# lucagem29/mcmc_clv_model

Measured on AMD Instinct MI355X. Metric: MCMC sweeps/sec x N_customers (customer-sweeps/s), higher is better.
Workload: dtype f64

## Files before the change

include/clvmcmc.h:

```cpp
#ifndef CLVMCMC_H
#define CLVMCMC_H

#include <stdint.h>

#ifdef __cplusplus
extern "C" {
#endif

#define CLV_ABI_VERSION 2

#define CLV_BLOCK 256
#define CLV_MAX_K 9
#define CLV_MAX_D 3

enum { CLV_OK = 0, CLV_EINVAL = -1, CLV_EHIP = -2, CLV_ESTATE = -3, CLV_ENOMEM = -4 };
enum { CLV_RNG_PHILOX = 0, CLV_RNG_REPLAY = 1 };
enum { CLV_SINK_FULL = 0, CLV_SINK_SUMMARY = 1, CLV_SINK_NONE = 2, CLV_SINK_SUMMARY_PCT = 3 };

#define CLV_SUMMARY_MU_CAP 0.05
enum {
  CLV_SUM_LAMBDA = 0, CLV_SUM_MU, CLV_SUM_Z, CLV_SUM_LOG_LAMBDA, CLV_SUM_LOG_MU,
  CLV_SUM_LAMBDA2, CLV_SUM_MU2, CLV_SUM_ETA, CLV_SUM_LOG_ETA, CLV_SUM_MU_CAPPED, CLV_SUM_TAU,
  CLV_N_SUM_STATS
};
// ... 88 lines not shown
                  int64_t sweeps_done);

int clv_set_timing(clv_sampler* s, int32_t enable);
int clv_kernel_time(clv_sampler* s, double* sweep_kernel_ms_total, int64_t* sweep_launches,
                    double* hyper_kernel_ms_total, int64_t* hyper_launches);

int clv_debug_host_times(const clv_sampler* s, int64_t* out);
int clv_debug_philox(uint32_t k0, uint32_t k1, const uint32_t* ctr, int64_t n, uint32_t* out);
int clv_debug_variates(uint64_t seed, int32_t chain, uint32_t sweep, int64_t n, int32_t n_steps,
                       float* t_l, float* t_m, float* u_acc, double* u_z, double* u_tau,
                       double* e_alive, double* eta_z, float* log2_u_acc);
int clv_debug_log2u_scan(uint64_t w_begin, uint64_t w_end, double* out);
int clv_debug_t3(const uint32_t* words, int64_t n, int32_t packed, float* t_l, float* t_m);
int clv_debug_level2(int32_t D, int32_t K, const clv_prior* prior, const double* xty,
                     const double* yty, const double* iw_normal, const double* iw_chi2,
                     const double* z, double* beta, double* sigma);
int clv_debug_stamps(clv_sampler* s, uint64_t* out);
int clv_debug_wg_stamps(clv_sampler* s, uint64_t* out);
int clv_debug_hyper_variates(uint64_t seed, int32_t chain, uint32_t sweep, double df, int64_t n,
                             double* chi2, double* normals);
int clv_debug_exp(const double* x, int64_t n, double* out);
int clv_debug_log(const double* x, int64_t n, double* out);
int clv_debug_mh_step(int64_t n, const int32_t* x, const uint8_t* z, const double* T_cal, const double* tau,
                      const double* mean, const double* prec3, const double* cur_pt, const float* t3,
                      const double* scale2, const float* log_u, double* out);
int clv_debug_wg_map(int32_t n_chains, int32_t nb, int32_t n_cu, int32_t* out);
int clv_debug_persist_fits(int64_t grid_wgs, int32_t blocks_per_cu, int32_t n_cu);
int clv_debug_persist_choice(int32_t D, int32_t K, int32_t n_chains, int64_t grid_wgs, int32_t blocks_per_cu,
                             int32_t n_cu);
int clv_debug_split_fits(int32_t n_chains, int32_t nb, int32_t blocks_per_cu, int32_t n_cu);
int clv_debug_split_choice(int32_t n_chains, int32_t nb, int32_t blocks_per_cu, int32_t n_cu);
int clv_debug_split_layout(int32_t n_chains, int32_t nb, int32_t* out);
int clv_debug_split_relay_plan(int32_t S, int32_t R, int32_t* out);
int clv_debug_split_stamps(clv_sampler* s, uint64_t* out);

enum { CLV_EXCHANGE_AUTO = 0, CLV_EXCHANGE_P2P = 1, CLV_EXCHANGE_COPY = 2 };
typedef struct clv_group clv_group;
int clv_group_create(clv_sampler* const* shards, int32_t n, int32_t exchange, clv_group** out);
int clv_group_run(clv_group* g, int64_t n_sweeps);
int32_t clv_group_exchange(const clv_group* g);
void clv_group_destroy(clv_group* g);

enum {
  CLV_L1_MEAN_LAMBDA = 0, CLV_L1_LAMBDA_P025, CLV_L1_LAMBDA_P975, CLV_L1_MEAN_MU, CLV_L1_MEAN_MU_CAPPED,
  CLV_L1_MU_P025, CLV_L1_MU_P975, CLV_L1_MEAN_Z, CLV_L1_MEAN_TAU, CLV_L1_MEAN_ETA, CLV_N_L1_STATS
};
int clv_predict(int32_t device, const double* level1, int64_t n_draws, int64_t n, int32_t width,
                const double* T_cal, double T_star, uint64_t seed, int32_t simulate_spend, double sigma_s,
                int64_t* x_future, double* spend_future);
int clv_predict_sampler(clv_sampler* s, double T_star, uint64_t seed, int32_t simulate_spend,
                        double sigma_s, int64_t* x_future, double* spend_future);
int clv_track(int32_t device, const double* level1, int64_t n_draws, int64_t n, int32_t width,
              const double* birth_week, const double* times, int32_t n_times, uint64_t seed,
              double* inc_weekly);
int clv_track_sampler(clv_sampler* s, const double* birth_week, const double* times, int32_t n_times,
                      uint64_t seed, double* inc_weekly);
int clv_level1_summary(int32_t device, const double* level1, int64_t n_draws, int64_t n, int32_t width,
                       double mu_cap, double* out);
int clv_level1_summary_sampler(clv_sampler* s, double mu_cap, double* out);
int clv_chain_total_loglik(int32_t device, const double* level1, int64_t n_draws, int64_t n, int32_t width,
                           const int32_t* x, const double* T_cal, double* mean_total);
int clv_chain_total_loglik_sampler(clv_sampler* s, double* mean_total);

enum {
  CLV_LTV_VALUE_MEAN = 0, CLV_LTV_VALUE_SD, CLV_LTV_VALUE_P025, CLV_LTV_VALUE_P50, CLV_LTV_VALUE_P975,
  CLV_LTV_RESIDUAL_MEAN, CLV_LTV_RESIDUAL_SD, CLV_LTV_RESIDUAL_P025, CLV_LTV_RESIDUAL_P50, CLV_LTV_RESIDUAL_P975,
// ... 109 lines not shown
```

mcmc_clv_model_amd/_lib.py:

```python
from __future__ import annotations

import ctypes
import os
from ctypes import c_uint8, POINTER, c_char_p, c_double, c_float, c_int32, c_int64, c_uint32, c_uint64, c_void_p

try:
    import torch
except Exception:
    torch = None

LIB_NAME = "libclvmcmc.so"
LIB_PATH = os.environ.get("CLV_LIB_PATH") or os.path.join(os.path.dirname(os.path.abspath(__file__)), LIB_NAME)

ABI_VERSION = 2
BLOCK = 256
MAX_K = 9
MAX_D = 3
RNG_PHILOX, RNG_REPLAY = 0, 1
SINK_FULL, SINK_SUMMARY, SINK_NONE, SINK_SUMMARY_PCT = 0, 1, 2, 3
EXCHANGE_AUTO, EXCHANGE_P2P, EXCHANGE_COPY = 0, 1, 2
SUM_STATS = ("lambda", "mu", "z", "log_lambda", "log_mu", "lambda2", "mu2", "eta", "log_eta", "mu_capped", "tau")
SUMMARY_MU_CAP = 0.05
N_SUM_STATS = len(SUM_STATS)
TAPE_HYPER = 40
# ... 62 lines not shown
        "clv_synchronize": (c_int32, [sp]),
        "clv_sweeps_done": (c_int64, [sp]),
        "clv_clock_ghz": (c_int32, [sp, POINTER(c_double)]),
        "clv_clock_probe": (c_int32, [sp, c_double, POINTER(c_double)]),
        "clv_launch_info": (c_int32, [sp, POINTER(c_int64)]),
        "clv_split_relay_steps": (c_int32, [sp, POINTER(c_int32)]),
        "clv_p2p_info": (c_int32, [sp, POINTER(c_int64)]),
        "clv_p2p_export": (c_int32, [sp, c_void_p]),
        "clv_p2p_connect": (c_int32, [sp, c_void_p, POINTER(c_uint64)]),
        "clv_p2p_disconnect": (c_int32, [sp]),
        "clv_p2p_set_persistent": (c_int32, [sp, c_int32]),
        "clv_set_wait_timeout": (c_int32, [sp, c_double]),
        "clv_set_stream": (c_int32, [sp, c_uint64]),
        "clv_note_sweeps": (c_int32, [sp, c_int64]),
        "clv_read_draws": (c_int32, [sp, dp, dp, dp]),
        "clv_stream_draws": (c_int32, [sp, dp]),
        "clv_read_summary": (c_int32, [sp, dp, POINTER(c_int64)]),
        "clv_get_state": (c_int32, [sp, dp, dp, dp]),
        "clv_set_state": (c_int32, [sp, dp, dp, dp, c_int64]),
        "clv_set_timing": (c_int32, [sp, c_int32]),
        "clv_kernel_time": (c_int32, [sp, dp, POINTER(c_int64), dp, POINTER(c_int64)]),
        "clv_debug_philox": (c_int32, [c_uint32, c_uint32, POINTER(c_uint32), c_int64, POINTER(c_uint32)]),
        "clv_debug_variates": (c_int32, [c_uint64, c_int32, c_uint32, c_int64, c_int32, POINTER(c_float),
                                         POINTER(c_float), POINTER(c_float), dp, dp, dp, dp, POINTER(c_float)]),
        "clv_debug_log2u_scan": (c_int32, [c_uint64, c_uint64, dp]),
        "clv_debug_host_times": (c_int32, [sp, POINTER(c_int64)]),
        "clv_debug_t3": (c_int32, [POINTER(c_uint32), c_int64, c_int32, POINTER(c_float), POINTER(c_float)]),
        "clv_debug_level2": (c_int32, [c_int32, c_int32, POINTER(ClvPrior), dp, dp, dp, dp, dp, dp, dp]),
        "clv_debug_hyper_variates": (c_int32, [c_uint64, c_int32, c_uint32, c_double, c_int64, dp, dp]),
        "clv_debug_stamps": (c_int32, [sp, POINTER(c_uint64)]),
        "clv_debug_wg_stamps": (c_int32, [sp, POINTER(c_uint64)]),
        "clv_debug_split_stamps": (c_int32, [sp, POINTER(c_uint64)]),
        "clv_debug_split_relay_plan": (c_int32, [c_int32, c_int32, POINTER(c_int32)]),
        "clv_debug_exp": (c_int32, [dp, c_int64, dp]),
        "clv_debug_log": (c_int32, [dp, c_int64, dp]),
        "clv_debug_mh_step": (c_int32, [c_int64, POINTER(c_int32), POINTER(c_uint8), dp, dp, dp, dp, dp,
                                        POINTER(c_float), dp, POINTER(c_float), dp]),
        "clv_debug_wg_map": (c_int32, [c_int32, c_int32, c_int32, POINTER(c_int32)]),
        "clv_debug_persist_choice": (c_int32, [c_int32, c_int32, c_int32, c_int64, c_int32, c_int32]),
        "clv_debug_persist_fits": (c_int32, [c_int64, c_int32, c_int32]),
        "clv_group_create": (c_int32, [POINTER(sp), c_int32, c_int32, POINTER(sp)]),
        "clv_group_run": (c_int32, [sp, c_int64]),
        "clv_group_exchange": (c_int32, [sp]),
        "clv_group_destroy": (None, [sp]),
        "clv_predict": (c_int32, [c_int32, dp, c_int64, c_int64, c_int32, dp, c_double, c_uint64, c_int32, c_double,
                                  POINTER(c_int64), dp]),
        "clv_predict_sampler": (c_int32, [sp, c_double, c_uint64, c_int32, c_double, POINTER(c_int64), dp]),
        "clv_track": (c_int32, [c_int32, dp, c_int64, c_int64, c_int32, dp, dp, c_int32, c_uint64, dp]),
        "clv_track_sampler": (c_int32, [sp, dp, dp, c_int32, c_uint64, dp]),
        "clv_level1_summary": (c_int32, [c_int32, dp, c_int64, c_int64, c_int32, c_double, dp]),
        "clv_level1_summary_sampler": (c_int32, [sp, c_double, dp]),
        "clv_chain_total_loglik": (c_int32, [c_int32, dp, c_int64, c_int64, c_int32, POINTER(c_int32), dp, dp]),
        "clv_chain_total_loglik_sampler": (c_int32, [sp, dp]),
        "clv_lifetime_value": (c_int32, [c_int32, dp, c_int64, c_int64, c_int32, dp, c_double, c_double, c_double,
                                         c_double, dp, dp]),
        "clv_lifetime_value_sampler": (c_int32, [sp, dp, c_double, c_double, c_double, c_double, dp, dp]),
        "clv_ltv_info": (c_int32, [POINTER(c_int64)]),
        "clv_pointwise_loglik": (c_int32, [c_int32, dp, c_int64, c_int64, c_int32, POINTER(c_int32), dp, dp, dp,
                                           c_double, dp]),
        "clv_psis_loo": (c_int32, [c_int32, dp, c_int64, c_int64, c_double, dp]),
        "clv_information_criteria": (c_int32, [c_int32, dp, c_int64, c_int64, c_int32, POINTER(c_int32), dp, dp, dp,
                                               c_double, c_double, dp]),
        "clv_information_criteria_sampler": (c_int32, [sp, c_int32, c_double, c_double, dp]),
        "clv_ic_info": (c_int32, [POINTER(c_int64)]),
        "clv_debug_information_criteria": (c_int32, [c_int32, dp, c_int64, c_int64, c_int32, POINTER(c_int32), dp,
                                                     dp, dp, c_double, c_double, c_int64, c_int32, dp]),
# ... 126 lines not shown
```

mcmc_clv_model_amd/csrc/capi.hip:

```cpp
#include <hip/hip_runtime.h>

#include <algorithm>
#include <chrono>
#include <cstdlib>
#include <cstdio>
#include <cstring>
#include <string>
#include <vector>

#include "internal.h"
#include "kernels.h"
#include "philox.h"

using namespace clv;

namespace {

thread_local std::string g_err;

constexpr int PRIOR_DOUBLES = 81 + 81 + 27 + 9;
constexpr int GRAPH_CHUNK = 64;
constexpr int TIMING_EVENTS = 256;

}
// ... 1556 lines not shown
  CLV_HIP(hipMemcpy(chi2, dc, sizeof(double) * n, hipMemcpyDeviceToHost));
  CLV_HIP(hipMemcpy(normals, dn, sizeof(double) * n, hipMemcpyDeviceToHost));
  CLV_HIP(hipFree(dc));
  CLV_HIP(hipFree(dn));
  return CLV_OK;
}

int clv_debug_persist_choice(int32_t D, int32_t K, int32_t n_chains, int64_t grid_wgs, int32_t blocks_per_cu,
                             int32_t n_cu) {
  return persist_grid_fits(grid_wgs, blocks_per_cu, n_cu) && persist_worth(D, K, n_chains, grid_wgs, n_cu) ? 1 : 0;
}

int clv_debug_persist_fits(int64_t grid_wgs, int32_t blocks_per_cu, int32_t n_cu) {
  return persist_grid_fits(grid_wgs, blocks_per_cu, n_cu) ? 1 : 0;
}

int clv_debug_split_fits(int32_t n_chains, int32_t nb, int32_t blocks_per_cu, int32_t n_cu) {
  return persist_split_fits(n_chains, nb, blocks_per_cu, n_cu) ? 1 : 0;
}

int clv_debug_split_choice(int32_t n_chains, int32_t nb, int32_t blocks_per_cu, int32_t n_cu) {
  return persist_split_fits(n_chains, nb, blocks_per_cu, n_cu) && persist_split_pays(n_chains, nb, n_cu) ? 1 : 0;
}

int clv_debug_split_relay_plan(int32_t S, int32_t R, int32_t* out) {
  if (!out || S < 0 || S > PRE_STEPS || !(R == 0 || R == 8 || R == 12)) return fail(CLV_EINVAL, "bad arguments");
  const SplitRelayPlan pl = split_relay_plan(S, R);
  const int32_t o[8] = {pl.own_begin, pl.own_end, pl.relay_begin, pl.relay_end,
                        pl.own_begin, pl.own_end, pl.relay_begin, pl.relay_end};
  std::copy(o, o + 8, out);
  return CLV_OK;
}

int clv_debug_split_layout(int32_t n_chains, int32_t nb, int32_t* out) {
  if (!out || n_chains < 1 || nb < 1 || nb > SPLIT_MAX_NB || n_chains >= (1 << 15)) return fail(CLV_EINVAL, "bad arguments");
  const std::vector<int32_t> m = persist_split_layout(n_chains, nb);
  const int nwg = split_wgs(nb);
  for (size_t i = 0; i < m.size(); ++i) {
    int32_t* o = out + 8 * i;
    const int p = m[i] & 0xFFFF;
    o[0] = m[i] >> 16;
    for (int k = 1; k < 8; ++k) o[k] = -1;
    if (p == nwg) continue;
    const int r0 = SPLIT_CW * p;
    o[1] = r0;
    o[2] = std::min(SPLIT_CW, 4 * nb - r0);
    const int b0 = (p & 1) ? (r0 - 2) / 4 : r0 / 4, b1 = (p & 1) ? (r0 + 2) / 4 : r0 / 4 + 1;
    o[3] = (p & 1) ? 3 : 1;
    o[4] = b0;
    if (b1 < nb) {
      o[5] = (p & 1) ? 1 : 2;
      o[6] = b1;
    }
    o[7] = (p & 1) ? nb + 2 * (b0 / 3) : -1;
  }
  return CLV_OK;
}

int clv_debug_wg_map(int32_t n_chains, int32_t nb, int32_t n_cu, int32_t* out) {
  if (!out || n_chains < 1 || nb < 0 || n_cu < 1 || n_chains >= (1 << 15) || nb >= (1 << 16))
    return fail(CLV_EINVAL, "bad arguments");
  const std::vector<int32_t> m = persist_wg_map(n_chains, nb, n_cu);
  std::copy(m.begin(), m.end(), out);
  return CLV_OK;
}

// ... 58 lines not shown
```

mcmc_clv_model_amd/csrc/kernels.h:

```cpp
#pragma once
#include <hip/hip_runtime.h>
#include <stdint.h>

#include "../../include/clvmcmc.h"

namespace clv {

constexpr int BLOCK = CLV_BLOCK;
constexpr int HS = 64;
constexpr int H_TAG = 63;
constexpr int TAPE_HYPER = 40;
constexpr int MAX_WORLD = 64;
constexpr int UMAIL = 2048;
constexpr int HV = 40;
constexpr int MAIL_TAIL = MAX_WORLD;
constexpr int CLK_RING = 1024;
constexpr int DIAG_WORDS = 16;
constexpr int PRE_STEPS = 20;
constexpr int SPLIT_CW = 6;
constexpr int SPLIT_NT = 512;
constexpr int SPLIT_MAX_NB = 256;
enum : int { LAYOUT_NONE = 0, LAYOUT_BLOCK = 1, LAYOUT_SPLIT = 2 };
__host__ __device__ inline int split_wgs(int nb) { return (2 * nb + 2) / 3; }
__host__ __device__ inline int split_records(int nb) { return nb + 2 * ((nb + 1) / 3); }
enum : int { WAIT_HYPER = 1, WAIT_BLOCKS = 2, WAIT_P2P_MAIL = 3, WAIT_FX_MAIL = 4, WAIT_RELAY = 5 };
#ifndef CLV_SPLIT_RELAY_STEPS
#define CLV_SPLIT_RELAY_STEPS 8
#endif
constexpr int SPLIT_RELAY_STEPS = CLV_SPLIT_RELAY_STEPS;
static_assert(SPLIT_RELAY_STEPS == 0 || SPLIT_RELAY_STEPS == 8 || SPLIT_RELAY_STEPS == 12, "relay point: 8 or 12 steps");
struct SplitRelayPlan {
  int own_begin, own_end, relay_begin, relay_end;
};
__host__ __device__ constexpr SplitRelayPlan split_relay_plan(int S, int R) {
  return SplitRelayPlan{0, (R > 0 && S > R) ? R : S, (R > 0 && S > R) ? R : S, S};
}

__host__ __device__ inline int64_t mail_slots(int world, int chains, int stride, int units_per_rank) {
  return 2LL * world * chains * stride * units_per_rank;
}

enum : int {
  H_BETA = 0,
  H_SIGMA = 27,
  H_P00 = 36, H_P01 = 37, H_P11 = 38,
  H_S00 = 39, H_S11 = 40,
  H_S22 = 41, H_POSTVAR = 42, H_SQRT_POSTVAR = 43, H_OMEGA2 = 44,
  H_INV_OMEGA2 = 45, H_INV_S22 = 46,
};

struct Ctrl {
  int64_t cur;
  uint32_t arrive;
  uint32_t abort;
};

struct Geometry {
  int D, K, S;
  int n_chains;
  int64_t n;
  int64_t n_global;
  int64_t shard_begin;
  int nb_local;
  int blocks_per_rank;
  int blocks_per_unit;
  int units_per_rank;
  int64_t n_units_global;
  int world_size;
// ... 127 lines not shown
```

mcmc_clv_model_amd/csrc/kernels.hip:

```cpp
#include <hip/hip_ext.h>

#include "fastmath.h"
#include "internal.h"
#include "kernels.h"
#include "philox.h"

#ifndef SWEEP_MH_PIPELINE
#define SWEEP_MH_PIPELINE 1
#endif
#ifndef CLV_OPAQUE_GI
#define CLV_OPAQUE_GI(D) ((D) == 3)
#endif
#ifndef CLV_L2_OPAQUE
#define CLV_L2_OPAQUE(P) (P)
#endif
#ifndef CLV_L2_LANE0_MAX
#define CLV_L2_LANE0_MAX 6
#endif
#ifndef PERSIST_REDUCE_GEN
#define PERSIST_REDUCE_GEN 1
#endif
#ifndef SWEEP_REDUCE_CHUNK
#define SWEEP_REDUCE_CHUNK 8
#endif
// ... 262 lines not shown
      v = lik;
    }
    return v;
  }
};

#ifdef CLV_STAMPS
__device__ __forceinline__ void stamp(unsigned long long* st, int64_t s, int k, bool is_min) {
  if (!st) return;
  const unsigned long long t = __builtin_amdgcn_s_memrealtime();
  unsigned long long* p = st + (s & 1023) * 8 + k;
  if (is_min) __hip_atomic_fetch_min(p, t, __ATOMIC_RELAXED, __HIP_MEMORY_SCOPE_AGENT);
  else __hip_atomic_fetch_max(p, t, __ATOMIC_RELAXED, __HIP_MEMORY_SCOPE_AGENT);
}
#define CLV_STAMP(st, s, k, is_min) stamp(st, s, k, is_min)
__device__ __forceinline__ void wg_stamp(unsigned long long* st, int64_t wg, int k) {
  if (!st) return;
  unsigned long long v;
  if (k < 2) v = __builtin_amdgcn_s_memrealtime();
  else if (k == 2) v = __builtin_amdgcn_s_getreg((4 << 0) | (0 << 6) | (31 << 11));
  else if (k == 3) v = __builtin_amdgcn_s_getreg((20 << 0) | (0 << 6) | (15 << 11));
  else v = __builtin_amdgcn_s_memtime();
  st[1024 * 8 + wg * 12 + k] = v;
}
#define CLV_WG_STAMP(st, wg, k) wg_stamp(st, wg, k)
#define CLV_P_STAMP(st, wg, k, on) \
  do {                             \
    if ((on) && (st)) (st)[1024 * 8 + (wg) * 12 + (k)] = (k) == 8 ? __builtin_amdgcn_s_getreg((4 << 0) | (0 << 6) | (31 << 11)) : (k) == 9 ? __builtin_amdgcn_s_getreg((20 << 0) | (0 << 6) | (15 << 11)) : __builtin_amdgcn_s_memrealtime(); \
  } while (0)
#define CLV_R_STAMP(a, wg, k, on)                                                                                       \
  do {                                                                                                                  \
    if ((on) && (a).stamps && (threadIdx.x & 63) == 0)                                                                  \
      (a).stamps[1024 * 8 + ((int64_t)(a).g.n_chains * ((a).g.nb_local + 1)) * 12 + (wg) * 16 + (k)] =                   \
          (k) >= 4 ? __builtin_amdgcn_s_getreg((4 << 0) | (0 << 6) | (31 << 11)) : __builtin_amdgcn_s_memrealtime();    \
  } while (0)
#else
#define CLV_R_STAMP(a, wg, k, on) ((void)0)
#define CLV_P_STAMP(st, wg, k, on) ((void)0)
#define CLV_WG_STAMP(st, wg, k) ((void)0)
#define CLV_STAMP(st, s, k, is_min) ((void)0)
#endif

__device__ __forceinline__ int64_t uniform_i64(int64_t v) {
  const uint32_t lo = __builtin_amdgcn_readfirstlane((uint32_t)v);
  const uint32_t hi = __builtin_amdgcn_readfirstlane((uint32_t)((uint64_t)v >> 32));
  return (int64_t)(((uint64_t)hi << 32) | lo);
}

__device__ __forceinline__ int64_t uniform64(int64_t x) {
  const uint32_t lo = __builtin_amdgcn_readfirstlane((uint32_t)x);
  const uint32_t hi = __builtin_amdgcn_readfirstlane((uint32_t)((uint64_t)x >> 32));
  return (int64_t)(((uint64_t)hi << 32) | lo);
}
__device__ __forceinline__ uint32_t stored_offset(int64_t s, const Geometry& g) {
  return (uint32_t)__builtin_amdgcn_readfirstlane((int32_t)(s - 1 - g.burnin));
}
__device__ __forceinline__ bool is_stored(int64_t s, const Geometry& g) {
  return s > g.burnin && s <= (int64_t)g.burnin + g.mcmc && stored_offset(s, g) % (uint32_t)g.thin == 0u;
}
__device__ __forceinline__ int64_t draw_index(int64_t s, const Geometry& g) {
  return (int64_t)(stored_offset(s, g) / (uint32_t)g.thin);
}

__global__ __launch_bounds__(64) void group_kernel(GroupArgs a) {
  const Geometry& g = a.g;
  const int u = blockIdx.x;
  const int c = blockIdx.y;
// ... 999 lines not shown
                                           const double* exp_tab) {
  constexpr int MC = MH_CHUNK_STEPS;
  S = opaque_uniform(S);
#pragma unroll
  for (int q = 0; q < NQ; ++q) {
    if (q * MC < S) {
      float2 t[MC];
      float u[MC];
#pragma unroll
      for (int st = 0; st < MC; ++st) {
        t[st] = v.t[(q * MC + st) * NT + v.lane];
        u[st] = v.u[(q * MC + st) * NT + v.lane];
      }
#pragma unroll
      for (int st = 0; st < MC; ++st) mh_step(cu, s00, s11, t[st].x, t[st].y, u[st], exp_tab);
    }
  }
}

template <int Q0, int Q1, int NT>
__device__ __forceinline__ void mh_pre_variates_range(const SlotPhilox& ph, int S_, const PreVariates& v) {
  constexpr int MC = MH_CHUNK_STEPS;
  const int S = opaque_uniform(S_);
#pragma unroll
  for (int q = Q0; q < Q1; ++q) {
    if (q * MC < S) {
      float tl[MC], tm[MC], lu[MC];
      mh_chunk_variates(ph, (uint32_t)q, tl, tm, lu);
#pragma unroll
      for (int st = 0; st < MC; ++st) {
        const int k = q * MC + st;
        v.t[k * NT + v.lane] = make_float2(tl[st], tm[st]);
        v.u[k * NT + v.lane] = k < S ? lu[st] : __builtin_inff();
      }
    }
  }
}
template <int Q0, int Q1, int NT, int D, int K, bool CL>
__device__ __forceinline__ void mh_run_pre_range(Cust<D, K, CL>& cu, const PreVariates& v, double s00, double s11, int S,
                                                 const double* exp_tab) {
  constexpr int MC = MH_CHUNK_STEPS;
  S = opaque_uniform(S);
#pragma unroll
  for (int q = Q0; q < Q1; ++q) {
    if (q * MC < S) {
      float2 t[MC];
      float u[MC];
#pragma unroll
      for (int st = 0; st < MC; ++st) {
        t[st] = v.t[(q * MC + st) * NT + v.lane];
        u[st] = v.u[(q * MC + st) * NT + v.lane];
      }
#pragma unroll
      for (int st = 0; st < MC; ++st) mh_step(cu, s00, s11, t[st].x, t[st].y, u[st], exp_tab);
    }
  }
}

template <int D>
struct CustOut {
  double lam, mu, eta, lgl, lgm, leta;
};

__device__ __forceinline__ double eta_normal(uint32_t k0, uint32_t k1, uint32_t gi, int64_t s, const double* tab) {
  const u32x4 r = customer_block(k0, k1, gi, (uint32_t)s, SLOT_ETA);
  return sqrt(-2.0 * log_fast(u53_open0(r.x, r.y), tab)) * cos2pi_u53(r.z, r.w, tab);
// ... 946 lines not shown
#ifndef CLV_SPLIT_HELP_CHUNKS
#define CLV_SPLIT_HELP_CHUNKS 2
#endif
constexpr int SPLIT_NC = SPLIT_CW * 64;
constexpr int SPLIT_PRE_LDS_BYTES = PRE_STEPS * SPLIT_NC * 12;

constexpr int RELAY_REC = 11;

template <int D, int K, int R>
__device__ __forceinline__ void split_relay_sweeps(const SweepArgs& a_launch, int64_t s_first, int64_t n_sweeps, int c,
                                                   int p, uint32_t k0, uint32_t k1, int64_t wgi, int64_t it_stamp,
                                                   double* parts, char* pool, double (*red)[K * D + D * (D + 1) / 2 + 1],
                                                   const double* exp_tab, double* Hs, uint32_t* s_abort) {
  constexpr int NS = K * D + D * (D + 1) / 2 + 1;
  constexpr int MC = MH_CHUNK_STEPS;
  constexpr int NQ = PRE_STEPS / MC;
  static_assert(R > 0 && R % MC == 0 && R < PRE_STEPS, "relay point: whole chunks, inside the pool");
  constexpr SplitRelayPlan PLAN = split_relay_plan(PRE_STEPS, R);
  static_assert(PLAN.own_begin == 0 && PLAN.own_end == PLAN.relay_begin && PLAN.own_end % MC == 0 && PLAN.relay_end == PRE_STEPS,
                "the relay plan cuts between chunks");
  static_assert(split_relay_plan(R + 1, R).own_end == PLAN.own_end, "one cut for every relayed S");
  constexpr int QR = PLAN.relay_begin / MC;
  __shared__ double relay_rec[RELAY_REC][128];
  __shared__ double relay_ret[4][128];
  __shared__ uint32_t relay_flag[2];
  __shared__ uint32_t relay_abort;
  (void)wgi;
  (void)it_stamp;
  const int tid = threadIdx.x;
  const int wave = __builtin_amdgcn_readfirstlane(tid >> 6);
  const bool first_wait = a_launch.pend_in != nullptr;
  if (tid < 2) relay_flag[tid] = 0;
  if (tid == 2) relay_abort = 0;

  if (wave >= SPLIT_CW) {
    const int rw = wave - SPLIT_CW;
    const int rl = tid - SPLIT_CW * 64;
    const PreVariates pv{(float2*)pool, (float*)(pool + PRE_STEPS * SPLIT_NC * 8), tid - 128};
    Cust<D, K> cu;
    {
      const Geometry& g = a_launch.g;
      const int64_t i = (int64_t)p * SPLIT_NC + (tid - 128);
      cu.active = i < g.n;
      cu.i = cu.active ? i : (g.n > 0 ? g.n - 1 : 0);
      cu.xr_[0] = 1.0;
#pragma unroll
      for (int k = 1; k < K; ++k) cu.xr_[k] = a_launch.cov[(int64_t)(k - 1) * g.n + cu.i];
      cu.gi = (uint32_t)(g.shard_begin + cu.i);
      cu.xm = 0.0;
      cu.lc.omz = 0.0;
      if (cu.active) mh_pre_variates_range<QR, NQ, SPLIT_NC>(SlotPhilox(k0, k1, cu.gi, (uint32_t)s_first), g.S, pv);
    }
    __syncthreads();
    for (int64_t it = 0; it < n_sweeps; ++it) {
      const SweepArgs& a = loop_args<CLV_PERSIST_FRESH_ARGS != 0>(a_launch);
      const Geometry& g = a.g;
      if (it > 0 || first_wait) {
        __syncthreads();
        if (*s_abort) return;
      }
      const int64_t s = uniform64(s_first + it);
      const bool stored = is_stored(s, g);
      const uint32_t tag = (uint32_t)it + 1u;
      bool seen = true;
      {
        const uint64_t t0 = __builtin_amdgcn_s_memrealtime();
        for (uint32_t poll = 0;; ++poll) {
          const uint32_t f = (uint32_t)__builtin_amdgcn_readfirstlane(
              (int)__hip_atomic_load(&relay_flag[rw], __ATOMIC_RELAXED, __HIP_MEMORY_SCOPE_WORKGROUP));
          if (f == tag) break;
          const int ws = wait_state(a, t0, poll, a.wait_ticks);
          if (ws != WAIT_GOING) {
            if (ws == WAIT_EXPIRED) {
              report_wait(a, WAIT_RELAY, s, c, false, p, 4 + rw, f, poll, t0);
              raise_abort(a);
            }
            if ((tid & 63) == 0) relay_abort = 1;
            seen = false;
            break;
          }
          __builtin_amdgcn_s_sleep(1);
        }
      }
      __builtin_amdgcn_fence(__ATOMIC_ACQUIRE, "workgroup", "local");
      CLV_R_STAMP(a, wgi, 2 * rw, it == it_stamp);
      StatGen<D, K> st{};
      __builtin_amdgcn_s_setprio(3);
      if (seen && cu.active) {
        cu.fc.A = relay_rec[0][rl];
        cu.fc.B = relay_rec[1][rl];
        cu.fc.C = relay_rec[2][rl];
        cu.fc.Dl = relay_rec[3][rl];
        cu.fc.El = relay_rec[4][rl];
        cu.fc.w = relay_rec[5][rl];
        cu.ll = relay_rec[6][rl];
        cu.lm = relay_rec[7][rl];
        cu.cur = relay_rec[8][rl];
        cu.lc.w = cu.fc.w;
        if (stored) {
          cu.xm = relay_rec[9][rl];
          cu.lc.omz = relay_rec[10][rl];
        }
        mh_run_pre_range<QR, NQ, SPLIT_NC>(cu, pv, Hs[H_S00], Hs[H_S11], g.S, exp_tab);
        const CustOut<D> out = cust_finish<D, K, false>(cu, a, s, stored, Hs, k0, k1, nullptr, exp_tab, st, nullptr);
        relay_ret[0][rl] = out.lam;
        relay_ret[1][rl] = out.mu;
        relay_ret[2][rl] = cu.ll;
        relay_ret[3][rl] = cu.lm;
      }
      wave_reduce_gen_row<NS, SWEEP_REDUCE_CHUNK>(st, red[4 + rw]);
      CLV_R_STAMP(a, wgi, 2 * rw + 1, it == it_stamp);
      __syncthreads();
      __builtin_amdgcn_s_setprio(0);
      if (relay_abort) return;
      if (cu.active && it + 1 < n_sweeps)
        mh_pre_variates_range<QR, NQ, SPLIT_NC>(SlotPhilox(k0, k1, cu.gi, (uint32_t)(s + 1)), g.S, pv);
    }
    return;
  }

  const bool relayed = wave >= 4;
  const int rl = tid - 4 * 64;
  const PreVariates pv{(float2*)pool, (float*)(pool + PRE_STEPS * SPLIT_NC * 8), tid};
  CLV_P_STAMP(a_launch.stamps, wgi, 7, tid == 0);
  Cust<D, K> cu;
  {
    const int64_t i = (int64_t)p * SPLIT_NC + tid;
    cu.active = i < a_launch.g.n;
    cu.i = cu.active ? i : (a_launch.g.n > 0 ? a_launch.g.n - 1 : 0);
  }
  cust_load(cu, a_launch, c);
  __syncthreads();
  if (cu.active) {
    cust_ztau<D, K, false>(cu, a_launch, s_first, k0, k1, nullptr, exp_tab);
    const SlotPhilox ph(k0, k1, cu.gi, (uint32_t)s_first);
    mh_pre_variates_range<0, QR, SPLIT_NC>(ph, a_launch.g.S, pv);
    if (!relayed) mh_pre_variates_range<QR, NQ, SPLIT_NC>(ph, a_launch.g.S, pv);
  }
  CLV_P_STAMP(a_launch.stamps, wgi, 10, tid == 0);
  for (int64_t it = 0; it < n_sweeps; ++it) {
    const SweepArgs& a = loop_args<CLV_PERSIST_FRESH_ARGS != 0>(a_launch);
    const Geometry& g = a.g;
    const double* hyp_c = a.hyp2 + (int64_t)c * HS;
    const int64_t s = uniform64(s_first + it);
    const bool stored = is_stored(s, g);
    const bool stp = tid == 0 && it == it_stamp;
    (void)stp;
    CLV_P_STAMP(a.stamps, wgi, 0, stp);
    if (it > 0 || first_wait) {
// ... 29 lines not shown
      if (cu.active) {
        cust_coeffs<D, K, false>(cu, Hs, exp_tab);
        mh_run_pre_range<0, QR, SPLIT_NC>(cu, pv, Hs[H_S00], Hs[H_S11], g.S, exp_tab);
        relay_rec[0][rl] = cu.fc.A;
        relay_rec[1][rl] = cu.fc.B;
        relay_rec[2][rl] = cu.fc.C;
        relay_rec[3][rl] = cu.fc.Dl;
        relay_rec[4][rl] = cu.fc.El;
        relay_rec[5][rl] = cu.fc.w;
        relay_rec[6][rl] = cu.ll;
        relay_rec[7][rl] = cu.lm;
        relay_rec[8][rl] = cu.cur;
        if (stored) {
          relay_rec[9][rl] = cu.xm;
          relay_rec[10][rl] = cu.lc.omz;
        }
      }
      __builtin_amdgcn_fence(__ATOMIC_RELEASE, "workgroup", "local");
      if ((tid & 63) == 0)
        __hip_atomic_store(&relay_flag[wave - 4], (uint32_t)it + 1u, __ATOMIC_RELAXED, __HIP_MEMORY_SCOPE_WORKGROUP);
    } else {
      __builtin_amdgcn_s_setprio(2);
      if (cu.active) {
        cust_coeffs<D, K, false>(cu, Hs, exp_tab);
        CLV_P_STAMP(a.stamps, wgi, 2, stp);
        mh_run_pre_range<0, QR, SPLIT_NC>(cu, pv, Hs[H_S00], Hs[H_S11], g.S, exp_tab);
        mh_run_pre_range<QR, NQ, SPLIT_NC>(cu, pv, Hs[H_S00], Hs[H_S11], g.S, exp_tab);
        CLV_P_STAMP(a.stamps, wgi, 3, stp);
        out = cust_finish<D, K, false>(cu, a, s, stored, Hs, k0, k1, nullptr, exp_tab, st, nullptr);
      }
      CLV_P_STAMP(a.stamps, wgi, 4, stp);
      wave_reduce_gen<NS, SWEEP_REDUCE_CHUNK>(st, red);
    }
    __syncthreads();
    if (relay_abort) return;
    {
      const int j = tid & 63;
      const int r0 = SPLIT_CW * p;
      if (j < NS && tid < 128) {
        if ((p & 1) == 0) {
          if (tid < 64) {
            st_wt(parts + (int64_t)(r0 / 4) * NS + j, ((red[0][j] + red[1][j]) + red[2][j]) + red[3][j]);
          } else {
            const int b = r0 / 4 + 1;
            if (b < g.nb_local) st_wt(parts + (int64_t)b * NS + j, red[4][j] + red[5][j]);
          }
        } else {
          if (tid < 64) {
            const int b = (r0 - 2) / 4;
            double* ext = parts + (int64_t)(g.nb_local + 2 * (b / 3)) * NS;
            st_wt(ext + j, red[0][j]);
            st_wt(ext + NS + j, red[1][j]);
          } else {
            const int b = (r0 + 2) / 4;
            if (b < g.nb_local) st_wt(parts + (int64_t)b * NS + j, ((red[2][j] + red[3][j]) + red[4][j]) + red[5][j]);
          }
        }
      }
    }
    __builtin_amdgcn_s_setprio(0);
    CLV_P_STAMP(a.stamps, wgi, 5, stp);
    CLV_P_STAMP(a.stamps, wgi, 8, stp);
    CLV_P_STAMP(a.stamps, wgi, 9, stp);
#ifdef CLV_STAMPS
    if (stp && a.stamps) a.stamps[1024 * 8 + wgi * 12 + 11] = blockIdx.y * gridDim.x + blockIdx.x;
#endif
    if (cu.active) {
      if (relayed) {
        cu.lam = relay_ret[0][rl];
        cu.mu = relay_ret[1][rl];
        out = CustOut<D>{cu.lam, cu.mu, 1.0, relay_ret[2][rl], relay_ret[3][rl], 0.0};
      }
      cust_store<D, K>(cu, out, a, c, s, stored, false);
      if (it + 1 < n_sweeps) {
        cust_ztau<D, K, false>(cu, a, s + 1, k0, k1, nullptr, exp_tab);
        const SlotPhilox ph(k0, k1, cu.gi, (uint32_t)(s + 1));
        mh_pre_variates_range<0, QR, SPLIT_NC>(ph, g.S, pv);
        if (!relayed) mh_pre_variates_range<QR, NQ, SPLIT_NC>(ph, g.S, pv);
      }
    }
    CLV_P_STAMP(a.stamps, wgi, 6, stp);
  }
  if (cu.active) {
    const int64_t ci = (int64_t)c * a_launch.g.n + cu.i;
    a_launch.lam_out[ci] = cu.lam;
    a_launch.mu_out[ci] = cu.mu;
  }
}

template <int D, int K, int HC, int R = 0>
__global__ __launch_bounds__(SPLIT_NT, 1) void persist_kernel_split(SweepArgs a, int64_t s_first, int64_t n_sweeps) {
  static_assert(D == 2, "the split layout is bivariate");
  constexpr int NXY = K * D;
  constexpr int NYY = D * (D + 1) / 2;
  constexpr int NS = NXY + NYY + 1;
  constexpr int MC = MH_CHUNK_STEPS;
  constexpr int NQ = PRE_STEPS / MC;
  static_assert(HC >= 0 && HC <= NQ, "helper share");
  __shared__ double red[SPLIT_CW][NS];
  __shared__ __attribute__((aligned(16))) double exp_tab[FAST_TAB_N];
  __shared__ double Hs[HS];
  __shared__ uint32_t s_abort;
  __shared__ __attribute__((aligned(16))) char pool[SPLIT_PRE_LDS_BYTES];
  const Geometry& g = a.g;
  const int nwg = split_wgs(g.nb_local);
  int c = blockIdx.y, p = blockIdx.x;
  if (a.wg_map) {
    const int32_t m = a.wg_map[blockIdx.y * gridDim.x + blockIdx.x];
    c = m >> 16;
    p = m & 0xFFFF;
// ... 752 lines not shown
```

Baseline: 11.00 billion.

## Let relay wavefronts pre-draw next-sweep MH variates during idle gaps

```diff
diff --git a/include/clvmcmc.h b/include/clvmcmc.h
--- a/include/clvmcmc.h
+++ b/include/clvmcmc.h
@@ -144,6 +144,7 @@
 int clv_debug_split_choice(int32_t n_chains, int32_t nb, int32_t blocks_per_cu, int32_t n_cu);
 int clv_debug_split_layout(int32_t n_chains, int32_t nb, int32_t* out);
 int clv_debug_split_relay_plan(int32_t S, int32_t R, int32_t* out);
+int clv_debug_split_draw_plan(int32_t R, int32_t share, int32_t* out);
 int clv_debug_split_stamps(clv_sampler* s, uint64_t* out);
 
 enum { CLV_EXCHANGE_AUTO = 0, CLV_EXCHANGE_P2P = 1, CLV_EXCHANGE_COPY = 2 };
diff --git a/mcmc_clv_model_amd/_lib.py b/mcmc_clv_model_amd/_lib.py
--- a/mcmc_clv_model_amd/_lib.py
+++ b/mcmc_clv_model_amd/_lib.py
@@ -118,6 +118,7 @@
         "clv_debug_wg_stamps": (c_int32, [sp, POINTER(c_uint64)]),
         "clv_debug_split_stamps": (c_int32, [sp, POINTER(c_uint64)]),
         "clv_debug_split_relay_plan": (c_int32, [c_int32, c_int32, POINTER(c_int32)]),
+        "clv_debug_split_draw_plan": (c_int32, [c_int32, c_int32, POINTER(c_int32)]),
         "clv_debug_exp": (c_int32, [dp, c_int64, dp]),
         "clv_debug_log": (c_int32, [dp, c_int64, dp]),
         "clv_debug_mh_step": (c_int32, [c_int64, POINTER(c_int32), POINTER(c_uint8), dp, dp, dp, dp, dp,
diff --git a/mcmc_clv_model_amd/csrc/capi.hip b/mcmc_clv_model_amd/csrc/capi.hip
--- a/mcmc_clv_model_amd/csrc/capi.hip
+++ b/mcmc_clv_model_amd/csrc/capi.hip
@@ -1612,6 +1612,23 @@
   return CLV_OK;
 }
 
+int clv_debug_split_draw_plan(int32_t R, int32_t share, int32_t* out) {
+  if (!out || !(R == 8 || R == 12) || share < -1 || share >= SPLIT_DRAW_SHARES) return fail(CLV_EINVAL, "bad arguments");
+  if (share < 0) {
+    out[0] = SPLIT_RELAY_DRAW;
+    return CLV_OK;
+  }
+  constexpr int NQ = PRE_STEPS / 4;
+  for (int row = 0; row < SPLIT_CW; ++row) {
+    for (int q = 0; q < NQ; ++q) {
+      const SplitDrawSlot d = split_draw_plan(R, share, row, q);
+      const int32_t o[4] = {d.wave, d.slot, d.staged, d.reader};
+      std::copy(o, o + 4, out + (row * NQ + q) * 4);
+    }
+  }
+  return CLV_OK;
+}
+
 int clv_debug_split_layout(int32_t n_chains, int32_t nb, int32_t* out) {
   if (!out || n_chains < 1 || nb < 1 || nb > SPLIT_MAX_NB || n_chains >= (1 << 15)) return fail(CLV_EINVAL, "bad arguments");
   const std::vector<int32_t> m = persist_split_layout(n_chains, nb);
diff --git a/mcmc_clv_model_amd/csrc/kernels.h b/mcmc_clv_model_amd/csrc/kernels.h
--- a/mcmc_clv_model_amd/csrc/kernels.h
+++ b/mcmc_clv_model_amd/csrc/kernels.h
@@ -34,6 +34,38 @@
 };
 __host__ __device__ constexpr SplitRelayPlan split_relay_plan(int S, int R) {
   return SplitRelayPlan{0, (R > 0 && S > R) ? R : S, (R > 0 && S > R) ? R : S, S};
+}
+#ifndef CLV_SPLIT_RELAY_DRAW
+#define CLV_SPLIT_RELAY_DRAW 4
+#endif
+#ifndef CLV_SPLIT_RELAY_GAP2_CHUNKS
+#define CLV_SPLIT_RELAY_GAP2_CHUNKS 3
+#endif
+#ifndef CLV_SPLIT_RELAY_GAP2_STOP
+#define CLV_SPLIT_RELAY_GAP2_STOP 6
+#endif
+constexpr int SPLIT_RELAY_DRAW = CLV_SPLIT_RELAY_DRAW;
+constexpr int SPLIT_RELAY_GAP2_CHUNKS = CLV_SPLIT_RELAY_GAP2_CHUNKS;
+constexpr int SPLIT_RELAY_GAP2_STOP = CLV_SPLIT_RELAY_GAP2_STOP;
+constexpr int SPLIT_DRAW_SHARES = 6;
+static_assert(SPLIT_RELAY_DRAW >= 0 && SPLIT_RELAY_DRAW < SPLIT_DRAW_SHARES, "draw share: 0..5");
+static_assert(SPLIT_RELAY_GAP2_CHUNKS >= 1 && SPLIT_RELAY_GAP2_STOP >= 1 && SPLIT_RELAY_GAP2_STOP <= SPLIT_CW, "gap 2 limits");
+enum : int { DRAW_WINDOW = 0, DRAW_GAP1 = 1, DRAW_GAP2 = 2 };
+struct SplitDrawSlot {
+  int wave;
+  int slot;
+  int staged;
+  int reader;
+};
+__host__ __device__ constexpr int split_draw_gap1_chunks(int share) { return share >= 4 ? share - 3 : share >= 2 ? share - 1 : 0; }
+__host__ __device__ constexpr SplitDrawSlot split_draw_plan(int R, int share, int row, int chunk) {
+  const int qr = R / 4;
+  const int reader = (row >= 4 && chunk >= qr) ? row + 2 : row;
+  if (share >= 1 && share <= 3 && row >= 4 && chunk >= qr && chunk < qr + SPLIT_RELAY_GAP2_CHUNKS)
+    return SplitDrawSlot{row + 2, DRAW_GAP2, 0, reader};
+  if ((row & 3) < 2 && chunk < split_draw_gap1_chunks(share) && chunk < qr)
+    return SplitDrawSlot{6 + (row & 1), DRAW_GAP1, 1, reader};
+  return SplitDrawSlot{reader, DRAW_WINDOW, 0, reader};
 }
 
 __host__ __device__ inline int64_t mail_slots(int world, int chains, int stride, int units_per_rank) {
diff --git a/mcmc_clv_model_amd/csrc/kernels.hip b/mcmc_clv_model_amd/csrc/kernels.hip
--- a/mcmc_clv_model_amd/csrc/kernels.hip
+++ b/mcmc_clv_model_amd/csrc/kernels.hip
@@ -318,7 +318,7 @@
   do {                                                                                                                  \
     if ((on) && (a).stamps && (threadIdx.x & 63) == 0)                                                                  \
       (a).stamps[1024 * 8 + ((int64_t)(a).g.n_chains * ((a).g.nb_local + 1)) * 12 + (wg) * 16 + (k)] =                   \
-          (k) >= 4 ? __builtin_amdgcn_s_getreg((4 << 0) | (0 << 6) | (31 << 11)) : __builtin_amdgcn_s_memrealtime();    \
+          (k) >= 4 && (k) < 12 ? __builtin_amdgcn_s_getreg((4 << 0) | (0 << 6) | (31 << 11)) : __builtin_amdgcn_s_memrealtime(); \
   } while (0)
 #else
 #define CLV_R_STAMP(a, wg, k, on) ((void)0)
@@ -1384,6 +1384,43 @@
         const int k = q * MC + st;
         v.t[k * NT + v.lane] = make_float2(tl[st], tm[st]);
         v.u[k * NT + v.lane] = k < S ? lu[st] : __builtin_inff();
+      }
+    }
+  }
+}
+template <int Q0, int Q1, int NT, int NS, bool COPY>
+__device__ __forceinline__ void mh_pre_variates_window(const SlotPhilox& ph, int S_, const PreVariates& v,
+                                                       const PreVariates& sv, uint32_t have) {
+  constexpr int MC = MH_CHUNK_STEPS;
+  const int S = opaque_uniform(S_);
+  have = (uint32_t)__builtin_amdgcn_readfirstlane((int)have);
+#pragma unroll
+  for (int q = Q0; q < Q1; ++q) {
+    if (q * MC < S) {
+      if ((have >> q) & 1u) {
+        if constexpr (COPY) {
+          float2 t[MC];
+          float u[MC];
+#pragma unroll
+          for (int st = 0; st < MC; ++st) {
+            t[st] = sv.t[(q * MC + st) * NS + sv.lane];
+            u[st] = sv.u[(q * MC + st) * NS + sv.lane];
+          }
+#pragma unroll
+          for (int st = 0; st < MC; ++st) {
+            v.t[(q * MC + st) * NT + v.lane] = t[st];
+            v.u[(q * MC + st) * NT + v.lane] = u[st];
+          }
+        }
+      } else {
+        float tl[MC], tm[MC], lu[MC];
+        mh_chunk_variates(ph, (uint32_t)q, tl, tm, lu);
+#pragma unroll
+        for (int st = 0; st < MC; ++st) {
+          const int k = q * MC + st;
+          v.t[k * NT + v.lane] = make_float2(tl[st], tm[st]);
+          v.u[k * NT + v.lane] = k < S ? lu[st] : __builtin_inff();
+        }
       }
     }
   }
@@ -2396,6 +2433,33 @@
   const bool first_wait = a_launch.pend_in != nullptr;
   if (tid < 2) relay_flag[tid] = 0;
   if (tid == 2) relay_abort = 0;
+  constexpr int DRAW = SPLIT_RELAY_DRAW;
+  constexpr int HC1 = split_draw_gap1_chunks(DRAW);
+  constexpr bool GAP2 = split_draw_plan(R, DRAW, 4, QR).slot == DRAW_GAP2;
+  static_assert(HC1 <= QR, "gap 1 draws owner chunks only");
+  static_assert(HC1 == 0 || (split_draw_plan(R, DRAW, 0, HC1 - 1).wave == SPLIT_CW && split_draw_plan(R, DRAW, 4, HC1 - 1).wave == SPLIT_CW &&
+                             split_draw_plan(R, DRAW, 1, HC1 - 1).wave == SPLIT_CW + 1 && split_draw_plan(R, DRAW, 5, HC1 - 1).wave == SPLIT_CW + 1 &&
+                             split_draw_plan(R, DRAW, 0, HC1).slot == DRAW_WINDOW && split_draw_plan(R, DRAW, 2, 0).slot == DRAW_WINDOW),
+                "gap 1: the first HC1 chunks of rows 0 and 4 by wavefront 6, of rows 1 and 5 by wavefront 7");
+  static_assert(GAP2 == (split_draw_plan(R, DRAW, 5, QR).slot == DRAW_GAP2) && split_draw_plan(R, DRAW, 4, QR - 1).slot != DRAW_GAP2,
+                "gap 2: the relay wavefront's own chunks, the same of rows 4 and 5");
+  constexpr int STAGE_STEPS = (HC1 > 0 ? HC1 : 1) * MC;
+  float2* stage_t = nullptr;
+  float* stage_u = nullptr;
+  uint32_t* relay_drawn = nullptr;
+  uint32_t* relay_arrive = nullptr;
+  if constexpr (HC1 > 0) {
+    __shared__ __attribute__((aligned(16))) char stage[4 * STAGE_STEPS * 64 * 12];
+    __shared__ uint32_t drawn[4];
+    stage_t = (float2*)stage;
+    stage_u = (float*)(stage + 4 * STAGE_STEPS * 64 * 8);
+    relay_drawn = drawn;
+  }
+  if constexpr (GAP2) {
+    __shared__ uint32_t arrive;
+    relay_arrive = &arrive;
+    if (tid == 3) arrive = 0;
+  }
 
   if (wave >= SPLIT_CW) {
     const int rw = wave - SPLIT_CW;
@@ -2426,6 +2490,45 @@
       const int64_t s = uniform64(s_first + it);
       const bool stored = is_stored(s, g);
       const uint32_t tag = (uint32_t)it + 1u;
+      const bool ahead = it + 1 < n_sweeps;
+      if constexpr (HC1 > 0) {
+        if (ahead) {
+          const int S = opaque_uniform(g.S);
+          uint32_t have[2] = {0u, 0u};
+          bool go = true;
+#pragma unroll
+          for (int q = 0; q < HC1; ++q) {
+#pragma unroll
+            for (int t = 0; t < 2; ++t) {
+              if (q * MC < S) {
+                if (go)
+                  go = (uint32_t)__builtin_amdgcn_readfirstlane(
+                           (int)__hip_atomic_load(&relay_flag[rw], __ATOMIC_RELAXED, __HIP_MEMORY_SCOPE_WORKGROUP)) != tag;
+                if (go) {
+                  const int64_t i = (int64_t)p * SPLIT_NC + (rw + 4 * t) * 64 + (tid & 63);
+                  if (i < g.n) {
+                    const SlotPhilox ph(k0, k1, (uint32_t)(g.shard_begin + i), (uint32_t)(s + 1));
+                    float tl[MC], tm[MC], lu[MC];
+                    mh_chunk_variates(ph, (uint32_t)q, tl, tm, lu);
+                    const int col = ((2 * t + rw) * STAGE_STEPS + q * MC) * 64 + (tid & 63);
+#pragma unroll
+                    for (int st = 0; st < MC; ++st) {
+                      stage_t[col + st * 64] = make_float2(tl[st], tm[st]);
+                      stage_u[col + st * 64] = q * MC + st < S ? lu[st] : __builtin_inff();
+                    }
+                  }
+                  have[t] |= 1u << q;
+                }
+              }
+            }
+          }
+          if ((tid & 63) == 0) {
+            relay_drawn[rw] = have[0];
+            relay_drawn[2 + rw] = have[1];
+          }
+        }
+        CLV_R_STAMP(a, wgi, 12 + rw, it == it_stamp);
+      }
       bool seen = true;
       {
         const uint64_t t0 = __builtin_amdgcn_s_memrealtime();
@@ -2474,11 +2577,49 @@
       }
       wave_reduce_gen_row<NS, SWEEP_REDUCE_CHUNK>(st, red[4 + rw]);
       CLV_R_STAMP(a, wgi, 2 * rw + 1, it == it_stamp);
-      __syncthreads();
-      __builtin_amdgcn_s_setprio(0);
-      if (relay_abort) return;
-      if (cu.active && it + 1 < n_sweeps)
-        mh_pre_variates_range<QR, NQ, SPLIT_NC>(SlotPhilox(k0, k1, cu.gi, (uint32_t)(s + 1)), g.S, pv);
+      if constexpr (GAP2) {
+        uint32_t have = 0u;
+        if (ahead) {
+          __builtin_amdgcn_s_setprio(0);
+          const int S = opaque_uniform(g.S);
+          const SlotPhilox ph(k0, k1, cu.gi, (uint32_t)(s + 1));
+          bool go = true;
+#pragma unroll
+          for (int q = QR; q < NQ; ++q) {
+            if (split_draw_plan(R, DRAW, 4, q).slot == DRAW_GAP2 && q * MC < S) {
+              if (go)
+                go = (int32_t)((uint32_t)__builtin_amdgcn_readfirstlane(
+                                   (int)__hip_atomic_load(relay_arrive, __ATOMIC_RELAXED, __HIP_MEMORY_SCOPE_WORKGROUP)) -
+                               ((tag - 1u) * (uint32_t)SPLIT_CW + (uint32_t)SPLIT_RELAY_GAP2_STOP)) < 0;
+              if (go) {
+                if (cu.active) {
+                  float tl[MC], tm[MC], lu[MC];
+                  mh_chunk_variates(ph, (uint32_t)q, tl, tm, lu);
+#pragma unroll
+                  for (int st = 0; st < MC; ++st) {
+                    const int k = q * MC + st;
+                    pv.t[k * SPLIT_NC + pv.lane] = make_float2(tl[st], tm[st]);
+                    pv.u[k * SPLIT_NC + pv.lane] = k < S ? lu[st] : __builtin_inff();
+                  }
+                }
+                have |= 1u << q;
+              }
+            }
+          }
+        }
+        CLV_R_STAMP(a, wgi, 14 + rw, it == it_stamp);
+        __syncthreads();
+        __builtin_amdgcn_s_setprio(0);
+        if (relay_abort) return;
+        if (cu.active && ahead)
+          mh_pre_variates_window<QR, NQ, SPLIT_NC, SPLIT_NC, false>(SlotPhilox(k0, k1, cu.gi, (uint32_t)(s + 1)), g.S, pv, pv, have);
+      } else {
+        __syncthreads();
+        __builtin_amdgcn_s_setprio(0);
+        if (relay_abort) return;
+        if (cu.active && ahead)
+          mh_pre_variates_range<QR, NQ, SPLIT_NC>(SlotPhilox(k0, k1, cu.gi, (uint32_t)(s + 1)), g.S, pv);
+      }
     }
     return;
   }
@@ -2574,6 +2715,9 @@
       CLV_P_STAMP(a.stamps, wgi, 4, stp);
       wave_reduce_gen<NS, SWEEP_REDUCE_CHUNK>(st, red);
     }
+    if constexpr (GAP2) {
+      if ((tid & 63) == 0) __hip_atomic_fetch_add(relay_arrive, 1u, __ATOMIC_RELAXED, __HIP_MEMORY_SCOPE_WORKGROUP);
+    }
     __syncthreads();
     if (relay_abort) return;
     {
@@ -2617,7 +2761,16 @@
       if (it + 1 < n_sweeps) {
         cust_ztau<D, K, false>(cu, a, s + 1, k0, k1, nullptr, exp_tab);
         const SlotPhilox ph(k0, k1, cu.gi, (uint32_t)(s + 1));
-        mh_pre_variates_range<0, QR, SPLIT_NC>(ph, g.S, pv);
+        if constexpr (HC1 > 0) {
+          const int w = __builtin_amdgcn_readfirstlane(tid >> 6);
+          const int sr = 2 * (w >> 2) + (w & 1);
+          const uint32_t have = (w & 3) < 2 ? relay_drawn[sr] : 0u;
+          const PreVariates sv{stage_t + sr * STAGE_STEPS * 64, stage_u + sr * STAGE_STEPS * 64, tid & 63};
+          mh_pre_variates_window<0, HC1, SPLIT_NC, 64, true>(ph, g.S, pv, sv, have);
+          mh_pre_variates_range<HC1, QR, SPLIT_NC>(ph, g.S, pv);
+        } else {
+          mh_pre_variates_range<0, QR, SPLIT_NC>(ph, g.S, pv);
+        }
         if (!relayed) mh_pre_variates_range<QR, NQ, SPLIT_NC>(ph, g.S, pv);
       }
     }
```

Result: faster. 11.46 billion, median of 6 (+4.2%).
